# mschoenb97/po2_quantization

Measured on AMD Instinct MI355X. Metric: quantized-conv fwd images/sec, ResNet56 224×224 bs=256; 1/2/4/8 MI355X, higher is better.
Workload: dtype fp32(bf16x3); 1 GPU; resnet56 quantized-conv chain: 56 fused po2-4bit quantize+conv fwd + head (stage-1 and stage-2 conv1->conv2 pairs as one launch each) (stride-2 conv1 + 1x1 shortcut of stages 2-3 as one launch each) (weight packs of the single-conv layers batched: one launch per 36); conv_pairs=True, conv_pairs_stage2=True, s2ds=True, pack_batch=True, autotune=True, image=224, batch_per_gpu=256, global_batch=256, quantizer=po2, bits=4, precision=bf16x3, parallelism=dp1, world_size=1, hip_graph=False

## Files before the change

### po2_quantization_amd/csrc/po2q_conv_pair.hip

```cpp
#include <hip/hip_runtime.h>

#include <algorithm>
#include <climits>
#include <cstdint>
#include <string>
#include <type_traits>
#ifdef PO2Q_PAIR_STAMPS
#include <cstdio>
#include <cstdlib>
#include <vector>
#endif

#include "../../include/po2q.h"
#include "po2q_epi.h"
#include "po2q_internal.h"
#include "po2q_quant_dev.h"
#include "po2q_rows_dev.h"
#include "po2q_x3_dev.h"

namespace po2q {

namespace {
template <int CC> constexpr int kQSW = 512 / CC;
template <int CC> constexpr int kQPlane = (kQSW<CC> + 2) * 2 * CC + 32;
// ... 403 lines not shown
#pragma unroll
                        for (int e = 0; e < 4; ++e) b4[e] = ok ? b4[e] : 0u;
                    }
                    uint2 h2, m2, l2;
                    split4p<false>(b4, h2, m2, l2);
                    const int wo = yoct<CC>(q + 1, (4 * nt + g) >> 1) + 8 * (g & 1);
                    *reinterpret_cast<uint2*>(yw + wo) = h2;
                    *reinterpret_cast<uint2*>(yw + YPL + wo) = m2;
                    *reinterpret_cast<uint2*>(yw + 2 * YPL + wo) = l2;
                }
            }
        }
        PO2Q_PSTAMP(7);
#ifdef PO2Q_PAIR_STAMPS
        ph_[8] += 1;
#endif
    };

    constexpr int MWW4 = 7 * SW / 4 + (RPAD ? 1 : 0);
    constexpr int MWD = (CC * MWW4 + 63) / 64;
    auto mw_row = [&](int jn) __attribute__((always_inline)) {
        const int h = p0 - 2 + jn;
        const bool hok = jn < nx && h >= 0 && h < a.H;
        const uint32_t roff = (uint32_t)(hok ? h : 0) * (uint32_t)a.W * 4u;
        const uint32_t base = raw_lds + (uint32_t)((jn % PD) * rawslot);
#pragma unroll
        for (int i = 0; i < MWD; ++i) {
            const int e = 64 * i + lane;
            const int c = e / MWW4, q = 4 * (e - c * MWW4);
            const uint32_t vo = (hok && c < CC && q < a.W) ? ((uint32_t)c * (uint32_t)HW + (uint32_t)q) * 4u + roff
                                                            : 0x7fffffffu;
            rows_dma16<(NTS & 2) != 0>(rs, vo, 0u, base + (uint32_t)i * 1024u);
        }
    };
    if constexpr (MW) {
        if (wave == nw) {
#pragma unroll
            for (int r = 0; r < PD - MWL; ++r) mw_row(r);
        }
    } else {
        const floatx4 z = floatx4{0.f, 0.f, 0.f, 0.f};
#pragma unroll
        for (int r = 0; r < PD - 1; ++r) {
            load_row(r, r);
#pragma unroll
            for (int i = 0; i < ST; ++i) rows_store<(NTS & 1) != 0>(ry, 0x7fffffffu, z);
        }
    }
    {
        unsigned* red = reinterpret_cast<unsigned*>(yr);
        unsigned* thr = red + 16;
        uint4* fr = reinterpret_cast<uint4*>(yr + 4096);
        static_assert(4096 + (WL2 ? 1 : 2) * NF * 64 * 16 <= 2 * yslot, "fragment scratch");
        scale1 = wq_prologue(a.q1, thr, red, nw + MW, fin1);
        wq_pack_rows_lds<CC>(a.q1, CC, CC, NT, KS, scale1, fin1, thr, fr, NF, CC == 16);
        scale2 = wq_prologue(a.q2, thr, red, nw + MW, fin2);
        if constexpr (WL2) {
            wq_pack_rows_lds<CC>(a.q2, CC, CC, NT, KS, scale2, fin2, thr, wl2, NF);
        } else {
            wq_pack_rows_lds<CC>(a.q2, CC, CC, NT, KS, scale2, fin2, thr, fr + NF * 64, NF, CC == 16);
#pragma unroll
            for (int f = 0; f < NF; ++f) bw2[WL2 ? 0 : f] = __builtin_bit_cast(bf16x8, fr[NF * 64 + f * 64 + lane]);
        }
#pragma unroll
        for (int f = 0; f < NF; ++f) bw1[f] = __builtin_bit_cast(bf16x8, fr[f * 64 + lane]);
#pragma unroll
        for (int nt = 0; nt < NT; ++nt) {
            if constexpr (E != 0) {
#pragma unroll
                for (int e = 0; e < 4; ++e) {
                    const int k1 = 16 * nt + 4 * (lane >> 4) + e;
                    bk1[nt * 4 + e] = a.b1 ? a.b1[k1] : 0.0f;
                    e1s[nt * 4 + e] = a.ps1 ? a.ps1[k1] : 1.0f;
                    e1b[nt * 4 + e] = a.pb1 ? a.pb1[k1] : 0.0f;
                }
            }
            const int k2 = 16 * nt + (lane & 15);
            bk2[nt] = (E && a.b2) ? a.b2[k2] : 0.0f;
            e2s[nt] = (E && a.ps2) ? a.ps2[k2] : 1.0f;
            e2b[nt] = (E && a.pb2) ? a.pb2[k2] : 0.0f;
        }
        asm volatile("s_waitcnt vmcnt(0)" ::: "memory");
#pragma unroll
        for (int nt = 0; nt < NT; ++nt) {
            if constexpr (E != 0) {
#pragma unroll
                for (int e = 0; e < 4; ++e) asm volatile("" : "+v"(bk1[nt * 4 + e]), "+v"(e1s[nt * 4 + e]), "+v"(e1b[nt * 4 + e]));
            }
            asm volatile("" : "+v"(bk2[nt]), "+v"(e2s[nt]), "+v"(e2b[nt]));
        }
#pragma unroll
        for (int f = 0; f < NF; ++f) asm volatile("" : "+v"(bw1[f]));
        if constexpr (!WL2) {
#pragma unroll
            for (int f = 0; f < NF; ++f) asm volatile("" : "+v"(bw2[WL2 ? 0 : f]));
        }
        if constexpr (E == 2) {
#pragma unroll
            for (int nt = 0; nt < NT; ++nt) {
#pragma unroll
                for (int e = 0; e < 4; ++e) {
                    const int c = nt * 4 + e;
                    e1b[c] = bk1[c] * e1s[c] + e1b[c];
                    e1s[c] = scale1 * e1s[c];
                }
                e2b[nt] = bk2[nt] * e2s[nt] + e2b[nt];
                e2s[nt] = scale2 * e2s[nt];
            }
        }
        __syncthreads();
        for (int e = tid; e < (2 * yslot) / 16; e += blockDim.x)
            reinterpret_cast<uint4*>(yr)[e] = make_uint4(0u, 0u, 0u, 0u);
        if (lane < 3 && wave < nw)
// ... 264 lines not shown
            if (i2 >= 0 && i2 < n1 && r2 >= 0 && r2 < a.H)
                mfmas(std::integral_constant<int, S>{}, std::false_type{}, yr + YR * yslot);
            else
                zero_slot(std::integral_constant<int, S>{});
        }
        const int o = j - 6;
        const bool orow = o >= 0 && o < rbe;
        const int g = lane >> 4;
        floatx4 vv[NG];
#pragma unroll
        for (int grp = 0; grp < NG; ++grp) {
            floatx4 v;
#pragma unroll
            for (int e = 0; e < 4; ++e)
                v[e] = E == 0 ? acc[D][grp][0][e] * scale + 0.0f
                       : E == 2 ? acc[D][grp][0][e] * es[0] + eb[0]
                                : (acc[D][grp][0][e] * scale + bk[0]) * es[0] + eb[0];
            if constexpr (E == 2) {
#pragma unroll
                for (int e = 0; e < 4; ++e) v[e] = v[e] < 0.0f ? 0.0f : v[e];
            } else if constexpr (E != 0) {
#pragma unroll
                for (int e = 0; e < 4; ++e) v[e] = epi_act(v[e], a.act2);
            }
            vv[grp] = v;
        }
        const bool hi8 = (lane & 8) != 0;
        floatx4 sa, sb;
#pragma unroll
        for (int e = 0; e < 4; ++e) {
            sa[e] = __int_as_float(__builtin_amdgcn_update_dpp(__float_as_int(vv[0][e]), __float_as_int(vv[NG - 1][e]),
                                                               0x128, 0xf, 0xc, false));
            sb[e] = __int_as_float(__builtin_amdgcn_update_dpp(__float_as_int(vv[NG - 1][e]), __float_as_int(vv[0][e]),
                                                               0x128, 0xf, 0x3, false));
        }
        const int q = q0 + (hi8 ? 16 : 0) + 4 * g;
        const uint32_t rowoff = (uint32_t)(orow ? p0 + o : 0) * a.W + (uint32_t)q;
        const uint32_t ca = (uint32_t)(lane & 7), cb = 8u + (uint32_t)(lane & 7);
        const bool ok = orow && q < a.W;
        rows_store<(NTS & 1) != 0>(ry, ok ? (ca * (uint32_t)HW + rowoff) * 4u : 0x7fffffffu, sa);
        rows_store<(NTS & 1) != 0>(ry, ok ? (cb * (uint32_t)HW + rowoff) * 4u : 0x7fffffffu, sb);
    };

    if (!roleA) {
#pragma unroll
        for (int r = 0; r < PD - 1; ++r) load_x(r, r);
    }
    {
        unsigned* red = reinterpret_cast<unsigned*>(yr);
        unsigned* thr = red + 16;
        uint4* fr = reinterpret_cast<uint4*>(yr + 4096);
        static_assert(4096 + 2 * NF * 64 * 16 <= 2 * yslot, "fragment scratch");
        bool fin1, fin2;
        const float scale1 = wq_prologue(a.q1, thr, red, 2 * NWR, fin1);
        wq_pack_rows_lds<CC>(a.q1, CC, CC, NT, KS, scale1, fin1, thr, fr, NF, true);
        const float scale2 = wq_prologue(a.q2, thr, red, 2 * NWR, fin2);
        wq_pack_rows_lds<CC>(a.q2, CC, CC, NT, KS, scale2, fin2, thr, fr + NF * 64, NF, true);
        const uint4* frw = fr + (roleA ? NF * 64 : 0);
#pragma unroll
        for (int f = 0; f < NF; ++f) bw[f] = __builtin_bit_cast(bf16x8, frw[f * 64 + lane]);
        scale = roleA ? scale2 : scale1;
        fin = roleA ? fin2 : fin1;
        if constexpr (E != 0) {
            const float *b = roleA ? a.b2 : a.b1, *ps = roleA ? a.ps2 : a.ps1, *pb = roleA ? a.pb2 : a.pb1;
#pragma unroll
            for (int e = 0; e < 4; ++e) {
                const int k = roleA ? (lane & 15) : 4 * (lane >> 4) + e;
                bk[e] = b ? b[k] : 0.0f;
                es[e] = ps ? ps[k] : 1.0f;
                eb[e] = pb ? pb[k] : 0.0f;
            }
        }
        asm volatile("s_waitcnt vmcnt(0)" ::: "memory");
        if constexpr (E != 0) {
#pragma unroll
            for (int c = 0; c < 4; ++c) asm volatile("" : "+v"(bk[c]), "+v"(es[c]), "+v"(eb[c]));
        }
#pragma unroll
        for (int f = 0; f < NF; ++f) asm volatile("" : "+v"(bw[f]));
        if constexpr (E == 2) {
#pragma unroll
            for (int c = 0; c < 4; ++c) {
                eb[c] = bk[c] * es[c] + eb[c];
                es[c] = scale * es[c];
            }
        }
        __syncthreads();
        for (int e = tid; e < (2 * yslot) / 16; e += blockDim.x)
            reinterpret_cast<uint4*>(yr)[e] = make_uint4(0u, 0u, 0u, 0u);
        if (lane < 3 && !roleA) *reinterpret_cast<uint4*>(slab + lane * PL + zero_off) = make_uint4(0u, 0u, 0u, 0u);
    }
    (void)fin;
    if (roleA) {
        for (int j = 0; j < nsteps; j += 6) {
            stepA(std::integral_constant<int, 0>{}, j);
            stepA(std::integral_constant<int, 1>{}, j + 1);
            stepA(std::integral_constant<int, 2>{}, j + 2);
            if (j + 3 >= nsteps) break;
            stepA(std::integral_constant<int, 3>{}, j + 3);
            stepA(std::integral_constant<int, 4>{}, j + 4);
            stepA(std::integral_constant<int, 5>{}, j + 5);
        }
    } else {
        for (int j = 0; j < nsteps; j += 6) {
            stepB(std::integral_constant<int, 0>{}, j);
            stepB(std::integral_constant<int, 1>{}, j + 1);
            stepB(std::integral_constant<int, 2>{}, j + 2);
            if (j + 3 >= nsteps) break;
            stepB(std::integral_constant<int, 3>{}, j + 3);
            stepB(std::integral_constant<int, 4>{}, j + 4);
            stepB(std::integral_constant<int, 5>{}, j + 5);
        }
    }
    asm volatile("s_waitcnt vmcnt(0)" ::: "memory");
}

static size_t pair_lds(int C, int waves, int pd, bool res, bool mw = false) {
    const int sw = 512 / C, wp = sw * waves;
    const int plane = (sw + 2) * 2 * C + 32;
    const int nf = 3 * (C == 16 ? 2 : 3) * (C / 16);
    const size_t slot = (mw && C == 16) ? ((size_t)C * (wp * 4 + 16) + 1023) / 1024 * 1024 : (size_t)C * wp * 4;
    return (size_t)pd * slot + 2 * 3 * (size_t)(7 * sw + 3) * 2 * C + (size_t)waves * 3 * plane +
           (res ? (size_t)waves * pd * kQResSlot : 0) + (C == 32 ? (size_t)nf * 64 * 16 : 0);
}

static bool pair_plan(PairPlan& pp, int N, int C, int H, int W, bool res, int pd, int nts, bool mw = false) {
    if (N <= 0 || H <= 0 || W <= 0 || W % 4 != 0 || (C != 16 && C != 32)) return false;
    const int sw = 512 / C;
    const int waves = (W + sw - 1) / sw;
    if (waves > 7) return false;
    if ((int64_t)C * H * W * 4 >= (1LL << 31)) return false;
    pp.C = C;
    pp.waves = waves;
    pp.pd = pd;
    pp.nts = nts;
    pp.lds = pair_lds(C, waves, pd, res, mw);
    if (pp.lds > 160 * 1024) return false;
    int nseg = std::max(1, (256 + N - 1) / N);
    nseg = std::min(nseg, std::max(1, H / 8));
    pp.RB = (H + nseg - 1) / nseg;
    pp.nseg = (H + pp.RB - 1) / pp.RB;
    const int64_t items = (int64_t)N * pp.nseg;
    if (items > INT_MAX / 2) return false;
    pp.blocks = (items + 7) / 8 * 8;
    return true;
// ... 279 lines not shown
```

### po2_quantization_amd/csrc/po2q_conv_pairw.hip

```cpp
#include <hip/hip_runtime.h>

#include <algorithm>
#include <climits>
#include <cstdint>
#include <cstdlib>
#include <string>
#include <type_traits>
#include <utility>

#include "../../include/po2q.h"
#include "po2q_epi.h"
#include "po2q_internal.h"
#include "po2q_quant_dev.h"
#include "po2q_rows_dev.h"
#include "po2q_x3_dev.h"

namespace po2q {

namespace {
constexpr int kPWC = 32;
constexpr int kPWSW = 32;
constexpr int kPWWaves = 4;
constexpr int kPWWp = kPWSW * kPWWaves;
constexpr int kPWPL = (kPWSW + 2) * 2 * kPWC + 32;
// ... 399 lines not shown
                    for (int e = 0; e < 4; ++e) v[e] += r[e];
                }
                if constexpr (E == 2) {
#pragma unroll
                    for (int e = 0; e < 4; ++e) v[e] = v[e] < 0.0f ? 0.0f : v[e];
                } else if constexpr (E != 0) {
#pragma unroll
                    for (int e = 0; e < 4; ++e) v[e] = epi_act(v[e], a.act2);
                }
                vv[grp] = v;
            }
            floatx4 sa, sb;
#pragma unroll
            for (int e = 0; e < 4; ++e) {
                sa[e] = __int_as_float(__builtin_amdgcn_update_dpp(__float_as_int(vv[0][e]), __float_as_int(vv[1][e]),
                                                                   0x128, 0xf, 0xc, false));
                sb[e] = __int_as_float(__builtin_amdgcn_update_dpp(__float_as_int(vv[1][e]), __float_as_int(vv[0][e]),
                                                                   0x128, 0xf, 0x3, false));
            }
            const uint32_t ca = (uint32_t)(16 * nt) + (uint32_t)(lane & 7), cb = ca + 8u;
            if constexpr ((DBG & 32) != 0) {
                if constexpr (S6 % 2 == 1) {
                    const uint32_t ro2 = rowoff >= (uint32_t)a.W ? rowoff - (uint32_t)a.W : rowoff;
                    rows_store<(NTS & 1) != 0>(ry, ok ? (ca * (uint32_t)HW + ro2) * 4u : 0x7fffffffu, sa);
                    rows_store<(NTS & 1) != 0>(ry, ok ? (ca * (uint32_t)HW + rowoff) * 4u : 0x7fffffffu, sa);
                    rows_store<(NTS & 1) != 0>(ry, ok ? (cb * (uint32_t)HW + ro2) * 4u : 0x7fffffffu, sb);
                    rows_store<(NTS & 1) != 0>(ry, ok ? (cb * (uint32_t)HW + rowoff) * 4u : 0x7fffffffu, sb);
                }
            } else if constexpr ((DBG & 4) == 0) {
                rows_store<(NTS & 1) != 0>(ry, ok ? (ca * (uint32_t)HW + rowoff) * 4u : 0x7fffffffu, sa);
                rows_store<(NTS & 1) != 0>(ry, ok ? (cb * (uint32_t)HW + rowoff) * 4u : 0x7fffffffu, sb);
            }
        }
    };

    if (!roleA) {
#pragma unroll
        for (int r = 0; r < (PIPE ? 2 : PD - 1); ++r) load_x(r, r);
    } else if constexpr (RES) {
        const floatx4 z = floatx4{0.f, 0.f, 0.f, 0.f};
#pragma unroll
        for (int r = 0; r < PD - 1; ++r) {
            load_res(r, r);
#pragma unroll
            for (int i = 0; i < ST; ++i) rows_store<(NTS & 1) != 0>(ry, 0x7fffffffu, z);
        }
    }
    {
        unsigned* red = reinterpret_cast<unsigned*>(yr);
        unsigned* thr = red + 16;
        uint4* fr = reinterpret_cast<uint4*>(yr + 4096);
        static_assert(4096 + 2 * NF * 64 * 16 <= 2 * yslot, "fragment scratch");
        bool fin1, fin2;
        const float scale1 = wq_prologue(a.q1, thr, red, 2 * kPWWaves, fin1);
        if constexpr ((DBG & 128) == 0) wq_pack_rows_lds<CC>(a.q1, CC, CC, NT, KS, scale1, fin1, thr, fr, NF);
        const float scale2 = wq_prologue(a.q2, thr, red, 2 * kPWWaves, fin2);
        if constexpr ((DBG & 128) == 0) {
            wq_pack_rows_lds<CC>(a.q2, CC, CC, NT, KS, scale2, fin2, thr, fr + NF * 64, NF);
            const uint4* frw = fr + (roleA ? NF * 64 : 0);
#pragma unroll
            for (int f = 0; f < NF; ++f) bw[f] = __builtin_bit_cast(bf16x8, frw[f * 64 + lane]);
        }
        scale = roleA ? scale2 : scale1;
        fin = roleA ? fin2 : fin1;
        if constexpr (E != 0) {
            const float *b = roleA ? a.b2 : a.b1, *ps = roleA ? a.ps2 : a.ps1, *pb = roleA ? a.pb2 : a.pb1;
#pragma unroll
            for (int nt = 0; nt < NT; ++nt)
#pragma unroll
                for (int e = 0; e < 4; ++e) {
                    const int k = roleA ? 16 * nt + (lane & 15) : 16 * nt + 4 * (lane >> 4) + e;
                    bk[nt * 4 + e] = b ? b[k] : 0.0f;
                    es[nt * 4 + e] = ps ? ps[k] : 1.0f;
                    eb[nt * 4 + e] = pb ? pb[k] : 0.0f;
                }
        }
        asm volatile("s_waitcnt vmcnt(0)" ::: "memory");
        if constexpr (E != 0) {
#pragma unroll
            for (int c = 0; c < NT * 4; ++c) asm volatile("" : "+v"(bk[c]), "+v"(es[c]), "+v"(eb[c]));
        }
#pragma unroll
        for (int f = 0; f < NF; ++f) asm volatile("" : "+v"(bw[f]));
        if constexpr (E == 2) {
#pragma unroll
            for (int c = 0; c < NT * 4; ++c) {
                eb[c] = bk[c] * es[c] + eb[c];
                es[c] = scale * es[c];
            }
        }
        if constexpr (E != 0) {
            if (roleA) {
#pragma unroll
                for (int nt = 0; nt < NT; ++nt) {
                    bk[nt] = bk[nt * 4];
                    es[nt] = es[nt * 4];
                    eb[nt] = eb[nt * 4];
                }
            }
        }
        __syncthreads();
        for (int e = tid; e < (2 * yslot) / 16; e += blockDim.x)
            reinterpret_cast<uint4*>(yr)[e] = make_uint4(0u, 0u, 0u, 0u);
        if constexpr (PIPE) {
            if (!roleA) {
                uint32_t bx[2][8], hx;
                raw_rd(raw, bx, hx);
                split_half(slab, 0, bx);
                split_half(slab, 1, bx);
                split_halo(slab, hx);
            }
        }
    }
    (void)fin;
    if constexpr ((DBG & 64) != 0) return;
    if (roleA) {
        for (int j = 0; j < nsteps; j += 6) {
            stepA(std::integral_constant<int, 0>{}, j);
            stepA(std::integral_constant<int, 1>{}, j + 1);
            stepA(std::integral_constant<int, 2>{}, j + 2);
            if (j + 3 >= nsteps) break;
            stepA(std::integral_constant<int, 3>{}, j + 3);
            stepA(std::integral_constant<int, 4>{}, j + 4);
            stepA(std::integral_constant<int, 5>{}, j + 5);
        }
    } else {
        for (int j = 0; j < nsteps; j += 6) {
            auto step = [&](auto S_, int jj) __attribute__((always_inline)) {
                if constexpr (PIPE) stepBP(S_, jj); else stepB(S_, jj);
            };
            step(std::integral_constant<int, 0>{}, j);
            step(std::integral_constant<int, 1>{}, j + 1);
            step(std::integral_constant<int, 2>{}, j + 2);
            if (j + 3 >= nsteps) break;
            step(std::integral_constant<int, 3>{}, j + 3);
            step(std::integral_constant<int, 4>{}, j + 4);
            step(std::integral_constant<int, 5>{}, j + 5);
        }
    }
    asm volatile("s_waitcnt vmcnt(0)" ::: "memory");
}

namespace {

size_t pairw_lds(int pd, bool res, bool pipe) {
    return (size_t)pd * kPWRaw + 2 * 3 * (size_t)kPWYPL + (size_t)kPWWaves * (pipe ? 2 : 1) * 3 * kPWPL +
           (res ? (size_t)kPWWaves * pd * kPWRes : 0);
}

template <int PD, int NTS>
hipError_t launch_pairw_t(int blocks, size_t lds, const PairWArgs& a, const float* x, float* y, bool res, bool pipe,
                          hipStream_t s) {
    const bool plain = !res && !a.b1 && !a.b2 && !a.ps1 && !a.pb1 && !a.ps2 && !a.pb2 && a.act1 == 0 && a.act2 == 0;
    const dim3 grid((unsigned)blocks), block(64 * 2 * kPWWaves);
#ifdef PO2Q_PAIRW_DIAG
    if (const char* dv = getenv("PO2Q_PAIR_W32_DBG")) {
        const int dbg = atoi(dv);
#define PO2Q_PWD(v) \
        if (dbg == v && plain && NTS == 3) { \
            hipLaunchKernelGGL((conv_pairw<PD, NTS, false, 0, false, v>), grid, block, lds, s, x, y, a); \
            return hipGetLastError(); \
        }
        PO2Q_PWD(9) PO2Q_PWD(11) PO2Q_PWD(13) PO2Q_PWD(15) PO2Q_PWD(25) PO2Q_PWD(29) PO2Q_PWD(27)
        PO2Q_PWD(31) PO2Q_PWD(64) PO2Q_PWD(192) PO2Q_PWD(128)
#undef PO2Q_PWD
    }
#endif
    if constexpr (PD == 2) {
// ... 75 lines not shown
```

### po2_quantization_amd/csrc/po2q_conv_rows2.hip

```cpp
#include <hip/hip_runtime.h>

#include <algorithm>
#include <climits>
#include <cstdint>
#include <cstdlib>
#include <string>
#include <type_traits>
#include <vector>

#include "../../include/po2q.h"
#include "po2q_epi.h"
#include "po2q_internal.h"
#include "po2q_quant_dev.h"
#include "po2q_rows_dev.h"
#include "po2q_x3_dev.h"

namespace po2q {

namespace {
constexpr int kR2EP = 17, kR2OP = 16;
template <int CC> constexpr int kR2Plane = (kR2EP + kR2OP) * 2 * CC + 32;
template <int CC> constexpr int kR2KS = CC == 16 ? 2 : 3;
}

// ... 192 lines not shown
            const unsigned char* rw = raw + RS * a.rawslot;
#pragma unroll
            for (int k = 0; k < NTASK; ++k) {
                uint32_t b8[8];
#pragma unroll
                for (int e = 0; e < 8; ++e) b8[e] = *reinterpret_cast<const uint32_t*>(rw + rd[k] + e * (a.W * 4));
                if (!tok[k]) {
#pragma unroll
                    for (int e = 0; e < 8; ++e) b8[e] = 0u;
                }
                uint4 hi, mid, lo;
                split3(b8, hi, mid, lo);
                *reinterpret_cast<uint4*>(slab + wa[k]) = hi;
                *reinterpret_cast<uint4*>(slab + PL + wa[k]) = mid;
                *reinterpret_cast<uint4*>(slab + 2 * PL + wa[k]) = lo;
            }
            if (lane < CC) {
                uint32_t hb = *reinterpret_cast<const uint32_t*>(rw + rd_h);
                hb = h_ok ? hb : 0u;
                uint16_t h16, m16, l16;
                split1(hb, h16, m16, l16);
                *reinterpret_cast<uint16_t*>(slab + wa_h) = h16;
                *reinterpret_cast<uint16_t*>(slab + PL + wa_h) = m16;
                *reinterpret_cast<uint16_t*>(slab + 2 * PL + wa_h) = l16;
            }
        }
        const int t = j >> 1;
        if constexpr ((S4 & 1) == 0) {
            constexpr int CUR = (S4 >> 1) & 1, PREV = CUR ^ 1;
            mfmas(std::integral_constant<int, 2>{}, std::integral_constant<int, PREV>{});
            mfmas(std::integral_constant<int, 0>{}, std::integral_constant<int, CUR>{});
            store_row(std::integral_constant<int, PREV>{}, t - 1, true);
            if constexpr (DS) ds_row(t, false);
        } else {
            constexpr int CUR = (S4 >> 1) & 1;
            mfmas(std::integral_constant<int, 1>{}, std::integral_constant<int, CUR>{});
            store_row(std::integral_constant<int, CUR>{}, t, false);
            if constexpr (DS) ds_row(t, true);
        }
    };

    {
        const floatx4 z = floatx4{0.f, 0.f, 0.f, 0.f};
#pragma unroll
        for (int r = 0; r < PD - 1; ++r) {
            load_row(r, r);
#pragma unroll
            for (int i = 0; i < ST; ++i) rows_store<(NTS & 1) != 0>(ry, 0x7fffffffu, z);
        }
    }
    {
        unsigned* red = reinterpret_cast<unsigned*>(planes);
        unsigned* thr = red + 16;
        scale = wq_prologue(a.q, thr, red, nw, fin);
        __syncthreads();
        wq_pack_rows_lds<CC>(a.q, K, CC, NT, KS, scale, fin, thr, wl, NF);
        if constexpr (DS) {
            __syncthreads();
            scaled = wq_prologue(a.qd, thr, red, nw, find);
            for (int e = tid; e < NT * 64; e += blockDim.x) {
                const int l = e & 63, nt = e >> 6, g = l >> 4, k = 16 * nt + (l & 15);
                const bool ok = CC == 32 || g >= 2;
                const int c0 = CC == 32 ? 8 * g : 8 * (g & 1);
                uint32_t h[8];
#pragma unroll
                for (int i = 0; i < 8; ++i)
                    h[i] = ok ? pack_one(a.qd.w[k * CC + c0 + i], scaled, find, a.qd.mode, a.qd.lo, a.qd.hi, thr) : 0u;
                wld[e] = make_uint4(h[0] | (h[1] << 16), h[2] | (h[3] << 16), h[4] | (h[5] << 16), h[6] | (h[7] << 16));
            }
#pragma unroll
            for (int nt = 0; nt < NT; ++nt) {
                const int k = 16 * nt + (lane & 15);
                epsd[nt] = (EPI && a.psd) ? a.psd[k] : 1.0f;
                epbd[nt] = (EPI && a.pbd) ? a.pbd[k] : 0.0f;
            }
        }
#pragma unroll
        for (int nt = 0; nt < NT; ++nt) {
            const int k = 16 * nt + (lane & 15);
            bk[nt] = bias ? bias[k] : 0.0f;
            eps_[nt] = (EPI && a.ps) ? a.ps[k] : 1.0f;
            epb_[nt] = (EPI && a.pb) ? a.pb[k] : 0.0f;
        }
        asm volatile("s_waitcnt vmcnt(0)" ::: "memory");
#pragma unroll
        for (int nt = 0; nt < NT; ++nt) asm volatile("" : "+v"(bk[nt]), "+v"(eps_[nt]), "+v"(epb_[nt]));
        if constexpr (DS) {
#pragma unroll
            for (int nt = 0; nt < NT; ++nt) asm volatile("" : "+v"(epsd[nt]), "+v"(epbd[nt]));
        }
        __syncthreads();
        if (lane < 3) *reinterpret_cast<uint4*>(slab + lane * PL + ZOFF) = make_uint4(0u, 0u, 0u, 0u);
    }
    for (int j = 0; j < nloop; j += 4) {
        step(std::integral_constant<int, 0>{}, j);
        step(std::integral_constant<int, 1>{}, j + 1);
        if (j + 2 >= nloop) break;
        step(std::integral_constant<int, 2>{}, j + 2);
        step(std::integral_constant<int, 3>{}, j + 3);
    }
    asm volatile("s_waitcnt vmcnt(0)" ::: "memory");
}

static size_t rows2_lds(int C, int waves, int pd, int rawslot) {
    const int nf = 3 * (C == 16 ? 2 : 3) * (2 * C / 16);
    const int plane = (kR2EP + kR2OP) * 2 * C + 32;
    return (size_t)nf * 1024 + (size_t)pd * rawslot + (size_t)waves * 3 * plane;
}

void rows2_candidates(const ConvPlan& b, int mode, int bits, int fsr, std::vector<PlanCand>& out) {
    if (mode == 0 || b.groups != 1) return;
    if (bits < 1 || bits > 16) return;
    const long lo = (long)fsr - (1L << (bits - 1)), hi = (long)fsr - 1;
    if (lo < -126 || hi > 127) return;
    if (b.R != 3 || b.S != 3 || b.sh != 2 || b.sw != 2 || b.ph != 1 || b.pw != 1 || b.dh != 1 || b.dw != 1) return;
    if (!((b.C == 16 && b.K == 32) || (b.C == 32 && b.K == 64))) return;
    if (b.W % 4 != 0 || b.Q % 4 != 0) return;
    const int waves = (b.Q + 15) / 16;
    if (waves < 1 || waves > 7 || 32 * waves < b.W) return;
    if ((int64_t)b.C * b.H * b.W * 4 >= (1LL << 31) || (int64_t)b.K * b.P * b.Q * 4 >= (1LL << 31)) return;
    if ((int64_t)b.K * b.C * 9 > 65536) return;
    ConvPlan p = b;
    p.kind = KIND_BF16X3_ROWS;
    p.vrx = 5;
    p.CC = b.C; p.NT = b.K / 16; p.NJ = 1; p.TQ = 16 * waves;
    p.steps = b.C == 16 ? 2 : 3; p.nchunks = 1; p.kblocks = 1; p.taps = 9;
    p.PS = 0; p.MI = 0; p.fp = 1;
    p.dma_d0 = p.dma_nck = p.dma_ni = p.dma_nw = p.dma_waves = p.dma_ov = 0;
    p.HH = 0; p.WW = p.WWp = 33;
    p.SB = 2 * b.C;
    p.plane = (kR2EP + kR2OP) * 2 * b.C + 32;
    p.packed_floats = (int64_t)3 * p.steps * p.NT * 64 * 4;
    p.tilesQ = 1;
    const int total4 = b.C * b.W / 4;
    const int ndma = (total4 + 64 * waves - 1) / (64 * waves);
    if (ndma < 1 || ndma > (b.C == 16 ? 2 : 4)) return;
    const int rawslot = std::max(b.C * b.W * 4, ndma * waves * 1024);
    p.dma_ni = ndma;
    p.dma_nck = rawslot;
    for (int pd : {2, 4}) {
        if (b.C == 32 && pd != 2) continue;
        ConvPlan q = p;
        q.pd = pd;
        q.lds_bytes = rows2_lds(b.C, waves, pd, rawslot);
        const int per_cu = std::min(2, (int)(160 * 1024 / q.lds_bytes));
        if (per_cu < 1) continue;
// ... 153 lines not shown
```

### po2_quantization_amd/csrc/po2q_conv_rowsf.hip

```cpp
#include <hip/hip_runtime.h>

#include <algorithm>
#include <climits>
#include <cstdlib>
#include <type_traits>
#include <vector>

#include "po2q_epi.h"
#include "po2q_internal.h"
#include "po2q_quant_dev.h"
#include "po2q_rows_dev.h"
#include "po2q_x3_dev.h"

namespace po2q {

namespace {
template <int CC> constexpr int kFSW = 512 / CC;
template <int CC> constexpr int kFWC = kFSW<CC> + 2;
template <int CC> constexpr int kFPlane = kFWC<CC> * CC * 2 + 32;
template <int CC> constexpr int kFKS = CC == 16 ? 2 : 3;
template <int CC> constexpr int kFWBytes = 3 * kFKS<CC> * (CC / 16) * 1024;
constexpr int kFResSlot = 2048;
constexpr int64_t kFusedStageMax = 65536;
}
// ... 206 lines not shown
#pragma unroll
                    for (int e = 0; e < 4; ++e) v[e] = outv(acc[D][grp][nt][e], nt);
                    if constexpr (RES) {
                        const floatx4 r = *reinterpret_cast<const floatx4*>(rres_row + ck * (SW * 4) + 4 * ql);
#pragma unroll
                        for (int e = 0; e < 4; ++e) v[e] = epi_act(v[e] + r[e], a.act);
                    }
                    rows_store<(NTS & 1) != 0>(ry, (orow && q < a.Q && !(DBG & 8)) ? (yk + (uint32_t)q) * 4u : 0x7fffffffu, v);
                }
            }
        } else {
            const int ch = lane & 15, g = lane >> 4;
#pragma unroll
            for (int grp = 0; grp < NG; ++grp) {
                floatx4 v;
#pragma unroll
                for (int e = 0; e < 4; ++e) v[e] = outv(acc[D][grp][0][e], 0);
                *reinterpret_cast<floatx4*>(slab + ch * 128 + 16 * ((4 * grp + g) ^ (ch & 7))) = v;
            }
#pragma unroll
            for (int i = 0; i < 2; ++i) {
                const int c = (lane >> 3) + 8 * i, b = lane & 7;
                floatx4 v = *reinterpret_cast<const floatx4*>(slab + c * 128 + 16 * (b ^ (c & 7)));
                if constexpr (RES) {
                    const floatx4 r = *reinterpret_cast<const floatx4*>(rres_row + c * 128 + 16 * b);
#pragma unroll
                    for (int e = 0; e < 4; ++e) v[e] = epi_act(v[e] + r[e], a.act);
                }
                const int q = q0 + 4 * b;
                const uint32_t yo = (uint32_t)c * (uint32_t)PQ + (uint32_t)(orow ? o : 0) * a.Q + q;
                rows_store<(NTS & 1) != 0>(ry, (orow && q < a.Q && !(DBG & 8)) ? yo * 4u : 0x7fffffffu, v);
            }
            if (lane == 0) *reinterpret_cast<uint4*>(slab + zero_off) = make_uint4(0u, 0u, 0u, 0u);
        }
#pragma unroll
        for (int grp = 0; grp < NG; ++grp)
#pragma unroll
            for (int nt = 0; nt < NT; ++nt) acc[D][grp][nt] = floatx4{0.f, 0.f, 0.f, 0.f};
    };

    {
        const floatx4 z = floatx4{0.f, 0.f, 0.f, 0.f};
#pragma unroll
        for (int r = 0; r < PD - 1; ++r) {
            load_row(r, r);
#pragma unroll
            for (int i = 0; i < ST; ++i) rows_store<(NTS & 1) != 0>(ry, 0x7fffffffu, z);
        }
    }
    {
        unsigned* red = reinterpret_cast<unsigned*>(raw + PD * rawslot);
        unsigned* thr = red + 16;
        if constexpr (FP) {
            scale = wq_prologue(a.q, thr, red, nw, fin);
            wq_pack_rows_lds<CC>(a.q, CC, CC, NT, KS, scale, fin, thr, wl, 3 * KS * NT);
        } else {
            for (int e = tid; e < 3 * KS * NT * 64; e += blockDim.x) wl[e] = wpk[e];
            scale = *scale_p;
        }
#pragma unroll
        for (int nt = 0; nt < NT; ++nt) {
            const int k = nt * 16 + (lane & 15);
            bk[nt] = bias ? bias[k] : 0.0f;
            eps_[nt] = (EPI && a.ps) ? a.ps[k] : 1.0f;
            epb_[nt] = (EPI && a.pb) ? a.pb[k] : 0.0f;
        }
        if constexpr (V & 1) {
#pragma unroll
            for (int f = 0; f < 3 * KS * NT; ++f) {
                if constexpr (FP)
                    bwr[f] = __builtin_bit_cast(bf16x8, wl[f * 64 + lane]);
                else
                    bwr[f] = __builtin_bit_cast(bf16x8, wpk[f * 64 + lane]);
            }
        }
        asm volatile("s_waitcnt vmcnt(0)" ::: "memory");
#pragma unroll
        for (int nt = 0; nt < NT; ++nt) asm volatile("" : "+v"(bk[nt]), "+v"(eps_[nt]), "+v"(epb_[nt]));
        if constexpr (V & 1) {
#pragma unroll
            for (int f = 0; f < 3 * KS * NT; ++f) asm volatile("" : "+v"(bwr[f]));
        }
        if (lane < 3) *reinterpret_cast<uint4*>(slab + lane * PL + zero_off) = make_uint4(0u, 0u, 0u, 0u);
        __syncthreads();
    }
    for (int j = 0; j < nrows; j += 6) {
        step(std::integral_constant<int, 0>{}, j);
        step(std::integral_constant<int, 1>{}, j + 1);
        step(std::integral_constant<int, 2>{}, j + 2);
        if (j + 3 >= nrows) break;
        step(std::integral_constant<int, 3>{}, j + 3);
        step(std::integral_constant<int, 4>{}, j + 4);
        step(std::integral_constant<int, 5>{}, j + 5);
    }
    asm volatile("s_waitcnt vmcnt(0)" ::: "memory");
}

static size_t rowsf_lds(int C, int waves, int pd) {
    const int plane = C == 16 ? kFPlane<16> : kFPlane<32>;
    const int wbytes = C == 16 ? kFWBytes<16> : kFWBytes<32>;
    const int sw = 512 / C;
    return (size_t)wbytes + (size_t)pd * C * (sw * waves) * 4 + (size_t)waves * 3 * plane;
}
static size_t rowsf_res_lds(const ConvPlan& p) { return p.lds_bytes + (size_t)(p.TQ / (512 / p.C)) * p.pd * kFResSlot; }

void rowsf_candidates(const ConvPlan& b, int mode, int bits, int fsr, std::vector<PlanCand>& out) {
    if (mode == 0 || b.groups != 1) return;
    if (bits < 1 || bits > 16) return;
// ... 155 lines not shown
```

### po2_quantization_amd/csrc/po2q_internal.h

```cpp
#pragma once
#include <hip/hip_runtime.h>

#include <cstddef>
#include <cstdint>
#include <string>
#include <vector>

namespace po2q {

void set_error(const std::string& msg);

constexpr int kThreads = 256;
constexpr int kMaxPartials = 1024;
constexpr int64_t kFusedAbsmaxMax = 1 << 20;

int absmax_blocks(int64_t n);

hipError_t launch_absmax(const float* w, int64_t n, unsigned* partial, int blocks, hipStream_t s);

hipError_t launch_quantize_plain(const float* w, int64_t n, const unsigned* partial, int nparts,
                                 int bits, int fsr, int mode, float* out, hipStream_t s);

inline bool is_lin_mode(int mode) { return mode == 3 || mode == 4; }
inline bool lin_bf16x3_ok(int bits, int num_iters, int groups) {
    return groups == 1 && bits >= 1 && bits <= 9 && num_iters >= 1;
}

enum ConvKind {
    KIND_MFMA_F32 = 0,
    KIND_DEPTHWISE = 1,
    KIND_BF16X3 = 2,
    KIND_BF16X3_DMA = 3,
    KIND_BF16X3_ROWS = 4,
    KIND_BF16X3_PW = 5,
    KIND_DIRECT_F32 = 6,
    KIND_PW_F32 = 7,
    KIND_BF16X3_IMG = 8,
    KIND_BF16X1 = 9,
    KIND_DW_BF16 = 10,
    KIND_BF16_ROWS = 11,
    KIND_BF16_ROWSK = 12
};

inline bool is_bf16x3_kind(int kind) {
    return kind == KIND_BF16X3 || kind == KIND_BF16X3_DMA || kind == KIND_BF16X3_ROWS || kind == KIND_BF16X3_PW ||
           kind == KIND_BF16X3_IMG;
}

struct ConvPlan {
    int N, C, H, W, K, R, S, sh, sw, ph, pw, dh, dw, groups;
    int P, Q, Cg, Kg;
    int kind;
    int MI, NJ;
    int NT;
    int TP, TQ, tilesP, tilesQ;
    int CC, nchunks, kblocks;
    int HH, WW, WWp, PS;
    int steps;
    int SB;
    int plane;
    int taps;
    int vrx;
    int pd;
    int nts;
    int fp = 0;
    int dma_d0, dma_nck, dma_ni, dma_nw;
    int dma_waves;
    int dma_ov;
    int64_t packed_floats;
    size_t lds_bytes;
    int64_t blocks;
};

bool plan_geometry(ConvPlan& p, int64_t N, int64_t C, int64_t H, int64_t W, int64_t K, int64_t R, int64_t S,
                   int64_t sh, int64_t sw, int64_t ph, int64_t pw, int64_t dh, int64_t dw, int64_t groups);

bool make_plan(ConvPlan& p, int64_t N, int64_t C, int64_t H, int64_t W, int64_t K, int64_t R,
               int64_t S, int64_t sh, int64_t sw, int64_t ph, int64_t pw, int64_t dh, int64_t dw,
               int64_t groups, int mode, int bits, int fsr, int flags);

bool plan_candidates(std::vector<ConvPlan>& out, int64_t N, int64_t C, int64_t H, int64_t W, int64_t K,
                     int64_t R, int64_t S, int64_t sh, int64_t sw, int64_t ph, int64_t pw, int64_t dh,
                     int64_t dw, int64_t groups, int mode, int bits, int fsr, int flags);

void tuned_store(const ConvPlan& p, int mode, int bits, int fsr, int flags);

struct WQuant {
    const float* w = nullptr;
    int n = 0;
    int lo = 0, hi = 0;
    int mode = 0;
};

hipError_t launch_conv_rows2(const ConvPlan& p, const float* x, const float* bias, float* y, hipStream_t s,
                             const float* ps, const float* pb, int act, bool epi, const WQuant& q,
                             float* yds = nullptr, const WQuant& qd = WQuant{}, const float* psd = nullptr,
                             const float* pbd = nullptr);

struct PlanCand {
    double cost;
    ConvPlan plan;
};

void x3_candidates(const ConvPlan& base, int mode, int bits, int fsr, std::vector<PlanCand>& out);
bool plan_bf16x3(ConvPlan& p, int mode, int bits, int fsr);

void x3p_candidates(const ConvPlan& base, std::vector<PlanCand>& out);
bool plan_bf16x3_dma(ConvPlan& p);

void rows_candidates(const ConvPlan& base, int mode, int bits, int fsr, std::vector<PlanCand>& out);

void pw_candidates(const ConvPlan& base, int mode, int bits, int fsr, std::vector<PlanCand>& out);
hipError_t launch_conv_pw(const ConvPlan& p, const float* x, const uint16_t* packed, const float* scale,
                          const float* bias, float* y, const float* ps, const float* pb, const float* res, int act,
                          hipStream_t s);

void img_candidates(const ConvPlan& base, int mode, int bits, int fsr, std::vector<PlanCand>& out);
hipError_t launch_conv_img(const ConvPlan& p, const float* x, const uint16_t* packed, const float* scale,
                           const float* bias, float* y, const float* ps, const float* pb, const float* res, int act,
                           hipStream_t s);

void f32s_candidates(const ConvPlan& base, std::vector<PlanCand>& out);
hipError_t launch_conv_f32s(const ConvPlan& p, const float* x, const float* w, const float* bias, float* y,
                            const float* ps, const float* pb, const float* res, int act, hipStream_t s);

hipError_t launch_pack_weights(const ConvPlan& p, const float* w, const unsigned* partial, int nparts,
                               int bits, int fsr, int mode, float* packed, hipStream_t s,
                               const float* delta = nullptr);

hipError_t launch_pack_bf16x3(const ConvPlan& p, const float* w, const unsigned* partial, int nparts,
                              int bits, int fsr, int mode, uint16_t* packed, float* scale_out,
                              hipStream_t s, const float* delta = nullptr);

struct PackReq {
    const ConvPlan* plan;
    const float* w;
    void* packed;
    float* scale;
    int bits, fsr, mode;
    unsigned* partial = nullptr;
    const float* delta = nullptr;
};
bool pack_batchable(const ConvPlan& p, int mode);
hipError_t launch_pack_batch(int n, const PackReq* reqs, hipStream_t s);
// ... 119 lines not shown
```

### po2_quantization_amd/csrc/po2q_quant_dev.h

```cpp
#pragma once
#include <hip/hip_runtime.h>

#include <cstdint>

#include "po2q_internal.h"
#include "po2q_thresholds.h"

namespace po2q {

__device__ __forceinline__ int decide_exponent(uint32_t b, int mode) {
    const int k = (b >= 0x00800000u) ? (int)(b >> 23) - 127 : (31 - (int)__clz(b)) - 149;
    return k + (b >= po2q_thr[mode][k - PO2Q_THR_KMIN] ? 1 : 0);
}

__device__ __forceinline__ bool exponent_of(float w, float scale, int mode, int lo, int hi, int& e) {
    const float nrm = w / scale;
    const uint32_t b = __float_as_uint(nrm) & 0x7fffffffu;
    if (b > 0x7f800000u) return false;
    int d;
    if (b == 0u) d = lo;
    else if (b < 0x3f800000u) d = decide_exponent(b, mode);
    else if (b == 0x3f800000u) d = 0;
    else d = hi;
    e = d < lo ? lo : (d > hi ? hi : d);
// ... 125 lines not shown
        const int c = rem / 9, tap = rem - c * 9;
        const int r = tap / 3, s = tap - r * 3;
        const uint16_t v = pack_one(q.w[i], scale, fin, q.mode, q.lo, q.hi, thr);
        int ks, grp;
        if (CC == 16) {
            ks = s == 2 ? 1 : 0;
            grp = (s == 2 ? 0 : 2 * s) + (c >> 3);
        } else {
            ks = (c >> 5) * 3 + s;
            grp = (c & 31) >> 3;
        }
        const int j = ((r * ksteps + ks) * NT + (k >> 4)) * 64 + (k & 15) + 16 * grp;
        h[j * 8 + (c & 7)] = v;
        if (CC == 16 && s == 2 && dup) h[(j + 32) * 8 + (c & 7)] = v;
    }
    __syncthreads();
}

template <int C>
__device__ __forceinline__ void wq_pack_tap_row_lds(const WQuant& q, int K, int CC, int NT, int ksteps, int r,
                                                    float scale, bool fin, const unsigned* thr, uint4* fr) {
    static_assert(C > 0, "channels");
    const int tid = threadIdx.x, nthr = (int)blockDim.x;
    const int nfr = ksteps * NT;
    for (int e = tid; e < nfr * 64; e += nthr) fr[e] = make_uint4(0u, 0u, 0u, 0u);
    __syncthreads();
    uint16_t* h = reinterpret_cast<uint16_t*>(fr);
    const int n = K * C * 3;
    for (int m = tid; m < n; m += nthr) {
        const int kc = m / 3, s = m - kc * 3;
        const int k = kc / C, c = kc - k * C;
        const uint16_t v = pack_one(q.w[kc * 9 + r * 3 + s], scale, fin, q.mode, q.lo, q.hi, thr);
        int ks, grp;
        if (CC == 16) {
            ks = s == 2 ? 1 : 0;
            grp = (s == 2 ? 0 : 2 * s) + (c >> 3);
        } else {
            ks = (c >> 5) * 3 + s;
            grp = (c & 31) >> 3;
        }
        const int j = (ks * NT + (k >> 4)) * 64 + (k & 15) + 16 * grp;
        h[j * 8 + (c & 7)] = v;
    }
    __syncthreads();
}

__device__ __forceinline__ float wq_prologue(const WQuant& q, unsigned* thr, unsigned* red, int nw, bool& fin) {
    for (int i = threadIdx.x; i < PO2Q_THR_COUNT; i += blockDim.x) thr[i] = po2q_thr[q.mode > 0 ? 1 : 0][i];
    const unsigned m = wq_absmax(q.w, q.n, red, nw);
    fin = (m > 0u) && (m < 0x7f800000u);
    return fin ? __uint_as_float(m) : 1.0f;
}

}
```

Baseline: 26900 images/s.

## Stage weight quantization in one pass with register-held float4 loads and merged reductions

Replaces the per-conv sequence of absmax prologue, sync and a separate pack pass with a single staged routine. It loads weights as float4 into registers, reduces the absmax for both convs of a pair (and the downsample weights) with one barrier, then packs from registers instead of re-reading global memory. This targets the serialized per-block weight-quantization prologue that every block repeats before its conv work. The cost is extra register pressure from holding NB float4s per tensor, plus a fallback to the old path for non-finite scales. An env var can turn it off, and a diagnostic probe can return early.

```diff
diff --git a/po2_quantization_amd/csrc/po2q_conv_pair.hip b/po2_quantization_amd/csrc/po2q_conv_pair.hip
--- a/po2_quantization_amd/csrc/po2q_conv_pair.hip
+++ b/po2_quantization_amd/csrc/po2q_conv_pair.hip
@@ -479,13 +479,25 @@
         unsigned* thr = red + 16;
         uint4* fr = reinterpret_cast<uint4*>(yr + 4096);
         static_assert(4096 + (WL2 ? 1 : 2) * NF * 64 * 16 <= 2 * yslot, "fragment scratch");
-        scale1 = wq_prologue(a.q1, thr, red, nw + MW, fin1);
-        wq_pack_rows_lds<CC>(a.q1, CC, CC, NT, KS, scale1, fin1, thr, fr, NF, CC == 16);
-        scale2 = wq_prologue(a.q2, thr, red, nw + MW, fin2);
-        if constexpr (WL2) {
-            wq_pack_rows_lds<CC>(a.q2, CC, CC, NT, KS, scale2, fin2, thr, wl2, NF);
+        constexpr int WNB = CC == 32 ? 6 : 2;
+        uint4* const fr2 = WL2 ? wl2 : fr + NF * 64;
+        if (wq_stage_on(a.q1)) {
+            unsigned* red2 = thr + PO2Q_THR_COUNT;
+            static_assert((16 + PO2Q_THR_COUNT + 16) * 4 <= 4096, "reduction scratch");
+            const WQuant* const qs[2] = {&a.q1, &a.q2};
+            uint4* const frs[2] = {fr, fr2};
+            float sc[2];
+            bool fn[2];
+            wq_stage_rows_lds<CC, WNB, 2>(qs, CC, CC, NT, KS, thr, red2, nw + MW, frs, NF, CC == 16, sc, fn);
+            scale1 = sc[0]; scale2 = sc[1];
+            fin1 = fn[0]; fin2 = fn[1];
         } else {
-            wq_pack_rows_lds<CC>(a.q2, CC, CC, NT, KS, scale2, fin2, thr, fr + NF * 64, NF, CC == 16);
+            scale1 = wq_prologue(a.q1, thr, red, nw + MW, fin1);
+            wq_pack_rows_lds<CC>(a.q1, CC, CC, NT, KS, scale1, fin1, thr, fr, NF, CC == 16);
+            scale2 = wq_prologue(a.q2, thr, red, nw + MW, fin2);
+            wq_pack_rows_lds<CC>(a.q2, CC, CC, NT, KS, scale2, fin2, thr, fr2, NF, CC == 16);
+        }
+        if constexpr (!WL2) {
 #pragma unroll
             for (int f = 0; f < NF; ++f) bw2[WL2 ? 0 : f] = __builtin_bit_cast(bf16x8, fr[NF * 64 + f * 64 + lane]);
         }
@@ -856,10 +868,23 @@
         uint4* fr = reinterpret_cast<uint4*>(yr + 4096);
         static_assert(4096 + 2 * NF * 64 * 16 <= 2 * yslot, "fragment scratch");
         bool fin1, fin2;
-        const float scale1 = wq_prologue(a.q1, thr, red, 2 * NWR, fin1);
-        wq_pack_rows_lds<CC>(a.q1, CC, CC, NT, KS, scale1, fin1, thr, fr, NF, true);
-        const float scale2 = wq_prologue(a.q2, thr, red, 2 * NWR, fin2);
-        wq_pack_rows_lds<CC>(a.q2, CC, CC, NT, KS, scale2, fin2, thr, fr + NF * 64, NF, true);
+        float scale1, scale2;
+        if (wq_stage_on(a.q1)) {
+            unsigned* red2 = thr + PO2Q_THR_COUNT;
+            static_assert((16 + PO2Q_THR_COUNT + 4 * NWR) * 4 <= 4096, "reduction scratch");
+            const WQuant* const qs[2] = {&a.q1, &a.q2};
+            uint4* const frs[2] = {fr, fr + NF * 64};
+            float sc[2];
+            bool fn[2];
+            wq_stage_rows_lds<CC, 1, 2>(qs, CC, CC, NT, KS, thr, red2, 2 * NWR, frs, NF, true, sc, fn);
+            scale1 = sc[0]; scale2 = sc[1];
+            fin1 = fn[0]; fin2 = fn[1];
+        } else {
+            scale1 = wq_prologue(a.q1, thr, red, 2 * NWR, fin1);
+            wq_pack_rows_lds<CC>(a.q1, CC, CC, NT, KS, scale1, fin1, thr, fr, NF, true);
+            scale2 = wq_prologue(a.q2, thr, red, 2 * NWR, fin2);
+            wq_pack_rows_lds<CC>(a.q2, CC, CC, NT, KS, scale2, fin2, thr, fr + NF * 64, NF, true);
+        }
         const uint4* frw = fr + (roleA ? NF * 64 : 0);
 #pragma unroll
         for (int f = 0; f < NF; ++f) bw[f] = __builtin_bit_cast(bf16x8, frw[f * 64 + lane]);
@@ -895,6 +920,9 @@
         if (lane < 3 && !roleA) *reinterpret_cast<uint4*>(slab + lane * PL + zero_off) = make_uint4(0u, 0u, 0u, 0u);
     }
     (void)fin;
+#ifdef PO2Q_WSTAGE_DIAG
+    if (a.q1.stage & 2) return;
+#endif
     if (roleA) {
         for (int j = 0; j < nsteps; j += 6) {
             stepA(std::integral_constant<int, 0>{}, j);
diff --git a/po2_quantization_amd/csrc/po2q_conv_pairw.hip b/po2_quantization_amd/csrc/po2q_conv_pairw.hip
--- a/po2_quantization_amd/csrc/po2q_conv_pairw.hip
+++ b/po2_quantization_amd/csrc/po2q_conv_pairw.hip
@@ -475,11 +475,27 @@
         uint4* fr = reinterpret_cast<uint4*>(yr + 4096);
         static_assert(4096 + 2 * NF * 64 * 16 <= 2 * yslot, "fragment scratch");
         bool fin1, fin2;
-        const float scale1 = wq_prologue(a.q1, thr, red, 2 * kPWWaves, fin1);
-        if constexpr ((DBG & 128) == 0) wq_pack_rows_lds<CC>(a.q1, CC, CC, NT, KS, scale1, fin1, thr, fr, NF);
-        const float scale2 = wq_prologue(a.q2, thr, red, 2 * kPWWaves, fin2);
+        float scale1, scale2;
+        constexpr int WNB = (CC * CC * 9 / 4 + 2 * kPWWaves * 64 - 1) / (2 * kPWWaves * 64);
+        const bool one_pass = (DBG & 128) == 0 && wq_stage_on(a.q1);
+        if (one_pass) {
+            unsigned* red2 = thr + PO2Q_THR_COUNT;
+            static_assert((16 + PO2Q_THR_COUNT + 4 * kPWWaves) * 4 <= 4096, "reduction scratch");
+            const WQuant* const qs[2] = {&a.q1, &a.q2};
+            uint4* const frs[2] = {fr, fr + NF * 64};
+            float sc[2];
+            bool fn[2];
+            wq_stage_rows_lds<CC, WNB, 2>(qs, CC, CC, NT, KS, thr, red2, 2 * kPWWaves, frs, NF, false, sc, fn);
+            scale1 = sc[0]; scale2 = sc[1];
+            fin1 = fn[0]; fin2 = fn[1];
+        } else {
+            scale1 = wq_prologue(a.q1, thr, red, 2 * kPWWaves, fin1);
+            if constexpr ((DBG & 128) == 0) wq_pack_rows_lds<CC>(a.q1, CC, CC, NT, KS, scale1, fin1, thr, fr, NF);
+            scale2 = wq_prologue(a.q2, thr, red, 2 * kPWWaves, fin2);
+            if constexpr ((DBG & 128) == 0)
+                wq_pack_rows_lds<CC>(a.q2, CC, CC, NT, KS, scale2, fin2, thr, fr + NF * 64, NF);
+        }
         if constexpr ((DBG & 128) == 0) {
-            wq_pack_rows_lds<CC>(a.q2, CC, CC, NT, KS, scale2, fin2, thr, fr + NF * 64, NF);
             const uint4* frw = fr + (roleA ? NF * 64 : 0);
 #pragma unroll
             for (int f = 0; f < NF; ++f) bw[f] = __builtin_bit_cast(bf16x8, frw[f * 64 + lane]);
@@ -537,6 +553,9 @@
     }
     (void)fin;
     if constexpr ((DBG & 64) != 0) return;
+#ifdef PO2Q_WSTAGE_DIAG
+    if (a.q1.stage & 2) return;
+#endif
     if (roleA) {
         for (int j = 0; j < nsteps; j += 6) {
             stepA(std::integral_constant<int, 0>{}, j);
diff --git a/po2_quantization_amd/csrc/po2q_conv_rows2.hip b/po2_quantization_amd/csrc/po2q_conv_rows2.hip
--- a/po2_quantization_amd/csrc/po2q_conv_rows2.hip
+++ b/po2_quantization_amd/csrc/po2q_conv_rows2.hip
@@ -268,10 +268,54 @@
     {
         unsigned* red = reinterpret_cast<unsigned*>(planes);
         unsigned* thr = red + 16;
-        scale = wq_prologue(a.q, thr, red, nw, fin);
-        __syncthreads();
-        wq_pack_rows_lds<CC>(a.q, K, CC, NT, KS, scale, fin, thr, wl, NF);
-        if constexpr (DS) {
+        constexpr int WNB = CC == 32 ? 6 : 3;
+        const bool one_pass = wq_stage_on(a.q) &&
+                              (!DS || (NT * 64 <= (int)blockDim.x && (a.q.mode > 0) == (a.qd.mode > 0)));
+        if (one_pass) {
+            float dv[8];
+            unsigned dm = 0u;
+            const int dg = tid >> 4 & 3;
+            const bool dok = DS && tid < NT * 64 && (CC == 32 || dg >= 2);
+            if constexpr (DS) {
+                const float* dw = a.qd.w + ((tid >> 6) * 16 + (tid & 15)) * CC + (CC == 32 ? 8 * dg : 8 * (dg & 1));
+                if (!dok) dw = a.qd.w;
+                if ((reinterpret_cast<uintptr_t>(a.qd.w) & 15u) == 0) {
+                    const float4 lo4 = reinterpret_cast<const float4*>(dw)[0], hi4 = reinterpret_cast<const float4*>(dw)[1];
+                    dv[0] = lo4.x; dv[1] = lo4.y; dv[2] = lo4.z; dv[3] = lo4.w;
+                    dv[4] = hi4.x; dv[5] = hi4.y; dv[6] = hi4.z; dv[7] = hi4.w;
+                } else {
+#pragma unroll
+                    for (int i = 0; i < 8; ++i) dv[i] = dw[i];
+                }
+#pragma unroll
+                for (int i = 0; i < 8; ++i) dm = max(dm, dok ? __float_as_uint(dv[i]) & 0x7fffffffu : 0u);
+            }
+            unsigned* red2 = thr + PO2Q_THR_COUNT;
+            const WQuant* const qs[1] = {&a.q};
+            uint4* const frs[1] = {wl};
+            float sc[1];
+            bool fn[1];
+            wq_stage_rows_lds<CC, WNB, 1>(qs, K, CC, NT, KS, thr, red2, nw, frs, NF, false, sc, fn,
+                                                   DS ? &dm : nullptr);
+            scale = sc[0];
+            fin = fn[0];
+            if constexpr (DS) {
+                find = (dm > 0u) && (dm < 0x7f800000u);
+                scaled = find ? __uint_as_float(dm) : 1.0f;
+                if (tid < NT * 64) {
+                    uint32_t h[8];
+#pragma unroll
+                    for (int i = 0; i < 8; ++i)
+                        h[i] = dok ? pack_one(dv[i], scaled, find, a.qd.mode, a.qd.lo, a.qd.hi, thr) : 0u;
+                    wld[tid] = make_uint4(h[0] | (h[1] << 16), h[2] | (h[3] << 16), h[4] | (h[5] << 16), h[6] | (h[7] << 16));
+                }
+            }
+        } else {
+            scale = wq_prologue(a.q, thr, red, nw, fin);
+            __syncthreads();
+            wq_pack_rows_lds<CC>(a.q, K, CC, NT, KS, scale, fin, thr, wl, NF);
+        }
+        if (DS && !one_pass) {
             __syncthreads();
             scaled = wq_prologue(a.qd, thr, red, nw, find);
             for (int e = tid; e < NT * 64; e += blockDim.x) {
@@ -284,6 +328,8 @@
                     h[i] = ok ? pack_one(a.qd.w[k * CC + c0 + i], scaled, find, a.qd.mode, a.qd.lo, a.qd.hi, thr) : 0u;
                 wld[e] = make_uint4(h[0] | (h[1] << 16), h[2] | (h[3] << 16), h[4] | (h[5] << 16), h[6] | (h[7] << 16));
             }
+        }
+        if constexpr (DS) {
 #pragma unroll
             for (int nt = 0; nt < NT; ++nt) {
                 const int k = 16 * nt + (lane & 15);
@@ -308,6 +354,9 @@
         __syncthreads();
         if (lane < 3) *reinterpret_cast<uint4*>(slab + lane * PL + ZOFF) = make_uint4(0u, 0u, 0u, 0u);
     }
+#ifdef PO2Q_WSTAGE_DIAG
+    if (a.q.stage & 2) return;
+#endif
     for (int j = 0; j < nloop; j += 4) {
         step(std::integral_constant<int, 0>{}, j);
         step(std::integral_constant<int, 1>{}, j + 1);
diff --git a/po2_quantization_amd/csrc/po2q_conv_rowsf.hip b/po2_quantization_amd/csrc/po2q_conv_rowsf.hip
--- a/po2_quantization_amd/csrc/po2q_conv_rowsf.hip
+++ b/po2_quantization_amd/csrc/po2q_conv_rowsf.hip
@@ -282,8 +282,19 @@
         unsigned* red = reinterpret_cast<unsigned*>(raw + PD * rawslot);
         unsigned* thr = red + 16;
         if constexpr (FP) {
-            scale = wq_prologue(a.q, thr, red, nw, fin);
-            wq_pack_rows_lds<CC>(a.q, CC, CC, NT, KS, scale, fin, thr, wl, 3 * KS * NT);
+            if (wq_stage_on(a.q)) {
+                const WQuant* const qs[1] = {&a.q};
+                uint4* const frs[1] = {wl};
+                float sc[1];
+                bool fn[1];
+                wq_stage_rows_lds<CC, 3, 1>(qs, CC, CC, NT, KS, thr, thr + PO2Q_THR_COUNT, nw, frs,
+                                                     3 * KS * NT, false, sc, fn);
+                scale = sc[0];
+                fin = fn[0];
+            } else {
+                scale = wq_prologue(a.q, thr, red, nw, fin);
+                wq_pack_rows_lds<CC>(a.q, CC, CC, NT, KS, scale, fin, thr, wl, 3 * KS * NT);
+            }
         } else {
             for (int e = tid; e < 3 * KS * NT * 64; e += blockDim.x) wl[e] = wpk[e];
             scale = *scale_p;
diff --git a/po2_quantization_amd/csrc/po2q_internal.h b/po2_quantization_amd/csrc/po2q_internal.h
--- a/po2_quantization_amd/csrc/po2q_internal.h
+++ b/po2_quantization_amd/csrc/po2q_internal.h
@@ -3,6 +3,7 @@
 
 #include <cstddef>
 #include <cstdint>
+#include <cstdlib>
 #include <string>
 #include <vector>
 
@@ -85,11 +86,21 @@
 
 void tuned_store(const ConvPlan& p, int mode, int bits, int fsr, int flags);
 
+static inline int wq_stage_default() {
+    const char* e = getenv("PO2Q_WSTAGE");
+    int v = (e && e[0] == '0') ? 0 : 1;
+#ifdef PO2Q_WSTAGE_DIAG
+    if (getenv("PO2Q_WSTAGE_PROBE")) v |= 2;
+#endif
+    return v;
+}
+
 struct WQuant {
     const float* w = nullptr;
     int n = 0;
     int lo = 0, hi = 0;
     int mode = 0;
+    int stage = wq_stage_default();
 };
 
 hipError_t launch_conv_rows2(const ConvPlan& p, const float* x, const float* bias, float* y, hipStream_t s,
diff --git a/po2_quantization_amd/csrc/po2q_quant_dev.h b/po2_quantization_amd/csrc/po2q_quant_dev.h
--- a/po2_quantization_amd/csrc/po2q_quant_dev.h
+++ b/po2_quantization_amd/csrc/po2q_quant_dev.h
@@ -201,4 +201,159 @@
     return fin ? __uint_as_float(m) : 1.0f;
 }
 
-}
+
+struct WSpan {
+    const float* w;
+    const float4* w4;
+    int head, n4, n;
+};
+
+__device__ __forceinline__ WSpan wq_span(const float* w, int n) {
+    WSpan s;
+    s.w = w;
+    s.n = n;
+    const int mis = (int)((reinterpret_cast<uintptr_t>(w) >> 2) & 3u);
+    s.head = min((4 - mis) & 3, n);
+    s.n4 = (n - s.head) >> 2;
+    s.w4 = reinterpret_cast<const float4*>(w + s.head);
+    return s;
+}
+
+__device__ __forceinline__ int wq_edge_index(const WSpan& s, int t) {
+    const int i = t < s.head ? t : 4 * s.n4 + t;
+    return (t < 6 && i < s.n) ? i : -1;
+}
+
+template <int NB>
+__device__ __forceinline__ void wq_load4(const WSpan& s, int base, float4 (&v)[NB]) {
+    const int tid = threadIdx.x, nthr = (int)blockDim.x;
+#pragma unroll
+    for (int u = 0; u < NB; ++u) v[u] = s.w4[min(base + u * nthr + tid, s.n4 - 1)];
+}
+
+template <int NB>
+__device__ __forceinline__ unsigned wq_max4(const float4 (&v)[NB], unsigned m) {
+#pragma unroll
+    for (int u = 0; u < NB; ++u) {
+        const unsigned a = __float_as_uint(v[u].x) & 0x7fffffffu, b = __float_as_uint(v[u].y) & 0x7fffffffu;
+        const unsigned c = __float_as_uint(v[u].z) & 0x7fffffffu, d = __float_as_uint(v[u].w) & 0x7fffffffu;
+        m = max(m, max(max(a, b), max(c, d)));
+    }
+    return m;
+}
+
+template <int C>
+__device__ __forceinline__ void wq_put_rows(uint16_t* h, int i, uint16_t v, int CC, int NT, int ksteps, bool dup) {
+    const int k = i / (C * 9), rem = i - k * (C * 9);
+    const int c = rem / 9, tap = rem - c * 9;
+    const int r = tap / 3, s = tap - r * 3;
+    int ks, grp;
+    if (CC == 16) {
+        ks = s == 2 ? 1 : 0;
+        grp = (s == 2 ? 0 : 2 * s) + (c >> 3);
+    } else {
+        ks = (c >> 5) * 3 + s;
+        grp = (c & 31) >> 3;
+    }
+    const int j = ((r * ksteps + ks) * NT + (k >> 4)) * 64 + (k & 15) + 16 * grp;
+    h[j * 8 + (c & 7)] = v;
+    if (CC == 16 && s == 2 && dup) h[(j + 32) * 8 + (c & 7)] = v;
+}
+
+template <int C, int NB>
+__device__ __forceinline__ void wq_pack4_rows(const WQuant& q, const WSpan& s, int base, const float4 (&v)[NB],
+                                              float edge, int CC, int NT, int ksteps, float scale,
+                                              const unsigned* thr, uint16_t* h, bool dup) {
+    const int tid = threadIdx.x, nthr = (int)blockDim.x;
+#pragma unroll
+    for (int u = 0; u < NB; ++u) {
+        const int i4 = base + u * nthr + tid;
+        if (i4 < s.n4) {
+            const float f[4] = {v[u].x, v[u].y, v[u].z, v[u].w};
+#pragma unroll
+            for (int e = 0; e < 4; ++e)
+                wq_put_rows<C>(h, s.head + 4 * i4 + e, pack_one(f[e], scale, true, q.mode, q.lo, q.hi, thr), CC, NT,
+                               ksteps, dup);
+        }
+    }
+    if (base == 0) {
+        const int ie = wq_edge_index(s, tid);
+        if (ie >= 0) wq_put_rows<C>(h, ie, pack_one(edge, scale, true, q.mode, q.lo, q.hi, thr), CC, NT, ksteps, dup);
+    }
+}
+
+__device__ __forceinline__ void wq_zero_lds(uint4* fr, int n) {
+    for (int e = threadIdx.x; e < n; e += (int)blockDim.x) fr[e] = make_uint4(0u, 0u, 0u, 0u);
+}
+
+__device__ __forceinline__ void wq_stage_thr(const WQuant& q, unsigned* thr) {
+    for (int i = threadIdx.x; i < PO2Q_THR_COUNT; i += blockDim.x) thr[i] = po2q_thr[q.mode > 0 ? 1 : 0][i];
+}
+
+__device__ __forceinline__ bool wq_stage_on(const WQuant& q) { return (q.stage & 1) != 0 && q.n >= 8; }
+
+template <int C, int NB, int NQ>
+__device__ __forceinline__ void wq_stage_rows_lds(const WQuant* const (&q)[NQ], int K, int CC, int NT, int ksteps,
+                                                  unsigned* thr, unsigned* red, int nw, uint4* const (&fr)[NQ],
+                                                  int nfr, bool dup, float (&scale)[NQ], bool (&fin)[NQ],
+                                                  unsigned* xm = nullptr) {
+    const int tid = threadIdx.x, nthr = (int)blockDim.x;
+    WSpan sp[NQ];
+    float4 v[NQ][NB];
+    float edge[NQ];
+#pragma unroll
+    for (int t = 0; t < NQ; ++t) {
+        sp[t] = wq_span(q[t]->w, q[t]->n);
+        wq_load4<NB>(sp[t], 0, v[t]);
+        const int ie = wq_edge_index(sp[t], tid);
+        edge[t] = ie >= 0 ? q[t]->w[ie] : 0.0f;
+    }
+    wq_stage_thr(*q[0], thr);
+#pragma unroll
+    for (int t = 0; t < NQ; ++t) wq_zero_lds(fr[t], nfr * 64);
+#pragma unroll
+    for (int t = 0; t < NQ; ++t) {
+        unsigned m = wq_max4<NB>(v[t], __float_as_uint(edge[t]) & 0x7fffffffu);
+        for (int base = NB * nthr; base < sp[t].n4; base += NB * nthr) {
+            float4 x[NB];
+            wq_load4<NB>(sp[t], base, x);
+            m = wq_max4<NB>(x, m);
+        }
+        m = wave_max_u32(m);
+        if ((tid & 63) == 0) red[t * nw + (tid >> 6)] = m;
+    }
+    if (xm) {
+        const unsigned m = wave_max_u32(*xm);
+        if ((tid & 63) == 0) red[NQ * nw + (tid >> 6)] = m;
+    }
+    __syncthreads();
+    if (xm) {
+        unsigned m = red[NQ * nw];
+        for (int i = 1; i < nw; ++i) m = max(m, red[NQ * nw + i]);
+        *xm = m;
+    }
+#pragma unroll
+    for (int t = 0; t < NQ; ++t) {
+        unsigned m = red[t * nw];
+        for (int i = 1; i < nw; ++i) m = max(m, red[t * nw + i]);
+        fin[t] = (m > 0u) && (m < 0x7f800000u);
+        scale[t] = fin[t] ? __uint_as_float(m) : 1.0f;
+    }
+#pragma unroll
+    for (int t = 0; t < NQ; ++t) {
+        if (!fin[t]) continue;
+        uint16_t* h = reinterpret_cast<uint16_t*>(fr[t]);
+        wq_pack4_rows<C, NB>(*q[t], sp[t], 0, v[t], edge[t], CC, NT, ksteps, scale[t], thr, h, dup);
+        for (int base = NB * nthr; base < sp[t].n4; base += NB * nthr) {
+            float4 x[NB];
+            wq_load4<NB>(sp[t], base, x);
+            wq_pack4_rows<C, NB>(*q[t], sp[t], base, x, 0.0f, CC, NT, ksteps, scale[t], thr, h, dup);
+        }
+    }
+    __syncthreads();
+#pragma unroll
+    for (int t = 0; t < NQ; ++t)
+        if (!fin[t]) wq_pack_rows_lds<C>(*q[t], K, CC, NT, ksteps, scale[t], false, thr, fr[t], nfr, dup);
+}
+
+}
```

After: 27070 images/s (median of 6 runs). Within noise of the previous version (+0.7%).
